# yondonfu/ai-rtc-agent

Measured on AMD Instinct MI355X. Metric: img2img FPS (SD-Turbo-class sd-turbo 512x512 1-step), higher is better.
Workload: dtype fp16; 1 GPU; model=sd-turbo (SD2.1-base UNet geometry, TAESD, 1-step), global_batch=1, resolution=512x512, parallelism=frame-level dp1, hip_graph=True

## Files before the change

### ai_rtc_agent_amd/ops/csrc/ext.cpp

```cpp

#include <torch/extension.h>
#include <ATen/cuda/CUDAContext.h>

#include "kernels.h"

#define CHECK_IN(x)                                                     \
  TORCH_CHECK(x.is_cuda(), #x " must be on GPU");                       \
  TORCH_CHECK(x.is_contiguous(), #x " must be contiguous")

namespace {

hipStream_t cur_stream() {
  return (hipStream_t)at::cuda::getCurrentCUDAStream().stream();
}

const uint16_t* h_ptr(const torch::Tensor& t) {
  return reinterpret_cast<const uint16_t*>(t.data_ptr<at::Half>());
}
uint16_t* h_ptr_mut(torch::Tensor& t) {
  return reinterpret_cast<uint16_t*>(t.data_ptr<at::Half>());
}

bool aligned16(const void* p) { return ((uintptr_t)p & 15) == 0; }

// ... 601 lines not shown
 public:
  VcnEncoder(int w, int h) : w_(w), h_(h) {
    char err[256] = {0};
    handle_ = airtc_vcn_enc_create(w, h, err, sizeof(err));
    if (!handle_) throw std::runtime_error(std::string("VCN encode: ") + err);
  }
  ~VcnEncoder() {
    if (handle_) airtc_vcn_enc_destroy(handle_);
  }
  VcnEncoder(const VcnEncoder&) = delete;
  pybind11::bytes encode(pybind11::bytes rgb, int qp) {
    std::string s(rgb);
    TORCH_CHECK((int)s.size() == w_ * h_ * 3, "rgb buffer size mismatch");
    std::vector<uint8_t> out((size_t)w_ * h_ * 2 + 65536);
    int n;
    {
      pybind11::gil_scoped_release nogil;
      n = airtc_vcn_enc_encode(handle_, (const uint8_t*)s.data(), qp,
                               out.data(), (int)out.size());
    }
    TORCH_CHECK(n > 0, "VCN encode failed rc=", n);
    return pybind11::bytes((const char*)out.data(), n);
  }

 private:
  void* handle_;
  int w_, h_;
};

pybind11::bytes h264_sps_pps(int width, int height) {
  uint8_t buf[256];
  int n = airtc_h264_sps_pps(width, height, buf, sizeof(buf));
  TORCH_CHECK(n > 0, "sps/pps generation failed");
  return pybind11::bytes(reinterpret_cast<const char*>(buf), n);
}

pybind11::dict vcn_probe() {
  char buf[512];
  int rc = airtc_vcn_probe(buf, sizeof(buf));
  pybind11::dict d;
  d["available"] = rc >= 0;
  d["h264_decode"] = rc >= 0 && (rc & 1);
  d["h264_encode"] = rc >= 0 && (rc & 2);
  d["detail"] = std::string(buf);
  return d;
}

torch::Tensor sched_add_noise(torch::Tensor x0, torch::Tensor noise,
                              torch::Tensor a, torch::Tensor bt) {
  CHECK_IN(x0);
  CHECK_IN(noise);
  TORCH_CHECK(x0.dtype() == torch::kHalf && noise.dtype() == torch::kHalf);
  TORCH_CHECK(a.dtype() == torch::kFloat && bt.dtype() == torch::kFloat);
  const long B = x0.size(0);
  TORCH_CHECK(a.numel() == B && bt.numel() == B, "coeffs must be (B,)");
  const long per_b = x0.numel() / B;
  TORCH_CHECK(per_b % 8 == 0, "row size must be a multiple of 8");
  auto out = torch::empty_like(x0);
  airtc_sched_add_noise(h_ptr(x0), h_ptr(noise), a.data_ptr<float>(),
                        bt.data_ptr<float>(), h_ptr_mut(out), per_b,
                        x0.numel(), cur_stream());
  return out;
}

torch::Tensor sched_blend(torch::Tensor xt, torch::Tensor eps,
                          torch::Tensor a, torch::Tensor bt,
                          torch::Tensor c_out, torch::Tensor c_skip) {
  CHECK_IN(xt);
  CHECK_IN(eps);
  TORCH_CHECK(xt.dtype() == torch::kHalf && eps.dtype() == torch::kHalf);
  const long B = xt.size(0);
  TORCH_CHECK(a.numel() == B && bt.numel() == B && c_out.numel() == B &&
              c_skip.numel() == B, "coeffs must be (B,)");
  const long per_b = xt.numel() / B;
  TORCH_CHECK(per_b % 8 == 0, "row size must be a multiple of 8");
  auto out = torch::empty_like(xt);
  airtc_sched_blend(h_ptr(xt), h_ptr(eps), a.data_ptr<float>(),
                    bt.data_ptr<float>(), c_out.data_ptr<float>(),
                    c_skip.data_ptr<float>(), h_ptr_mut(out), per_b,
                    xt.numel(), cur_stream());
  return out;
}

torch::Tensor rcfg_apply(int64_t mode, torch::Tensor eps, torch::Tensor coef,
                         c10::optional<torch::Tensor> delta,
                         c10::optional<torch::Tensor> stock, int64_t fbs) {
  CHECK_IN(eps);
  CHECK_IN(coef);
  TORCH_CHECK(mode >= 0 && mode <= 2, "mode must be 0 (self), 1 (initialize) or 2 (full)");
  TORCH_CHECK(eps.dtype() == torch::kHalf && coef.dtype() == torch::kFloat);
  TORCH_CHECK(eps.dim() >= 1 && fbs >= 1);
  const long B = coef.numel();
  const long rows_in = mode == 0 ? B : (mode == 1 ? B + fbs : 2 * B);
  TORCH_CHECK(B >= 1 && eps.size(0) == rows_in, "eps has ", eps.size(0),
              " rows, mode ", mode, " with ", B, " coefficient rows needs ",
              rows_in);
  TORCH_CHECK(fbs <= B && B % fbs == 0, "fbs must divide the row count");
  const long per_b = eps.numel() / rows_in;
  auto shape = eps.sizes().vec();
  shape[0] = B;
  auto out = torch::empty(shape, eps.options());
  auto overlap = [](const torch::Tensor& a, const torch::Tensor& b) {
    const char* a0 = static_cast<const char*>(a.data_ptr());
    const char* b0 = static_cast<const char*>(b.data_ptr());
    return a0 < b0 + b.nbytes() && b0 < a0 + a.nbytes();
  };
  TORCH_CHECK(!overlap(out, eps), "out must not alias eps");
  const float* dp = nullptr;
  uint16_t* sp = nullptr;
  bool vec = per_b % 8 == 0 && aligned16(eps.data_ptr()) &&
             aligned16(out.data_ptr());
  if (mode != 2) {
    TORCH_CHECK(delta.has_value() && stock.has_value(),
                "self/initialize need delta and stock");
    CHECK_IN((*delta));
    CHECK_IN((*stock));
    TORCH_CHECK(delta->dtype() == torch::kFloat && delta->numel() == B,
                "delta must be f32 (B,)");
    TORCH_CHECK(stock->dtype() == torch::kHalf && stock->sizes() == out.sizes(),
                "stock must be f16 with the output's shape");
    TORCH_CHECK(!overlap(*stock, eps), "stock must not alias eps");
    TORCH_CHECK(!overlap(out, *stock), "out must not alias stock");
    dp = delta->data_ptr<float>();
    sp = h_ptr_mut(*stock);
    vec = vec && aligned16(sp);
  }
  if (out.numel() == 0) return out;
  airtc_rcfg_apply((int)mode, h_ptr(eps), sp, coef.data_ptr<float>(), dp,
                   h_ptr_mut(out), B, fbs, per_b, vec ? 1 : 0, cur_stream());
  return out;
}

torch::Tensor conv2d_fp8(torch::Tensor x, torch::Tensor w_fp8,
                         torch::Tensor dq, double a_scale,
                         c10::optional<torch::Tensor> bias,
                         c10::optional<torch::Tensor> cbias,
                         c10::optional<torch::Tensor> residual, int64_t R,
                         int64_t S, int64_t stride, int64_t pad, int64_t act,
                         c10::optional<torch::Tensor> in_affine,
                         int64_t in_act, double out_scale) {
  CHECK_IN(x);
  CHECK_IN(w_fp8);
  CHECK_IN(dq);
  const bool x_q8 = x.dtype() == torch::kUInt8;
  TORCH_CHECK(x_q8 || x.dtype() == torch::kHalf,
              "x must be f16 or u8 e4m3 codes");
  TORCH_CHECK(w_fp8.dtype() == torch::kUInt8, "w_fp8 must be e4m3 bytes");
  TORCH_CHECK(dq.dtype() == torch::kFloat, "dq must be f32[OC]");
  const int B = x.size(0), H = x.size(1), W = x.size(2), IC = x.size(3);
  const int OC = w_fp8.size(0);
  TORCH_CHECK(IC % 64 == 0, "fp8 conv path requires IC % 64 == 0");
  TORCH_CHECK(dq.numel() == OC, "dq must have OC entries");
  TORCH_CHECK(w_fp8.size(1) == (long)R * S * IC, "w_fp8 must be (OC, R*S*IC)");
  TORCH_CHECK(!(x_q8 && in_affine.has_value()),
              "pre-quantized input cannot take a fused input affine");
  const int HO = (H + 2 * (int)pad - (int)R) / (int)stride + 1;
  const int WO = (W + 2 * (int)pad - (int)S) / (int)stride + 1;
  int path0 = airtc_conv2d_splitk_for(B, HO, WO, OC, IC);
  if (path0 == 0) path0 = HO * WO >= 2048 ? 1 : -1;
  const int splitk0 = path0 > 0 ? path0 : -path0;
  const bool want_q8 = out_scale > 0 && splitk0 == 1;
  auto out = torch::empty({B, HO, WO, OC},
                          x.options().dtype(want_q8 ? torch::kUInt8
                                                    : torch::kHalf));
  const float* bp = nullptr;
  if (bias.has_value()) {
    TORCH_CHECK(bias->dtype() == torch::kFloat && bias->is_contiguous());
    bp = bias->data_ptr<float>();
  }
  const uint16_t* cb = nullptr;
  if (cbias.has_value()) {
    CHECK_IN((*cbias));
    TORCH_CHECK(cbias->dtype() == torch::kHalf);
    cb = h_ptr(*cbias);
  }
  const uint16_t* res = nullptr;
  if (residual.has_value()) {
    CHECK_IN((*residual));
    TORCH_CHECK(residual->dtype() == torch::kHalf);
    TORCH_CHECK(residual->numel() == out.numel(), "residual shape mismatch");
    res = h_ptr(*residual);
  }
  const float* aff = nullptr;
  if (in_affine.has_value()) {
    CHECK_IN((*in_affine));
    TORCH_CHECK(in_affine->dtype() == torch::kFloat &&
                    in_affine->numel() == (long)B * IC * 2,
                "in_affine must be (B, IC, 2) f32");
    aff = in_affine->data_ptr<float>();
  }
  const int path = path0;
  const int splitk = splitk0;
  float* wsp = nullptr;
  torch::Tensor ws;
  if (splitk > 1) {
    ws = torch::empty({(long)B * splitk, (long)HO * WO, OC},
                      x.options().dtype(torch::kFloat));
    wsp = ws.data_ptr<float>();
  }
  const uint16_t* xp = x_q8
                           ? reinterpret_cast<const uint16_t*>(
                                 x.data_ptr<uint8_t>())
                           : h_ptr(x);
  uint16_t* op = want_q8 ? nullptr : h_ptr_mut(out);
  uint8_t* oq = want_q8 ? out.data_ptr<uint8_t>() : nullptr;
  airtc_conv2d_fp8_mfma(xp, w_fp8.data_ptr<uint8_t>(),
                        dq.data_ptr<float>(), bp, cb, res, op, wsp,
                        B, H, W, IC, HO, WO, OC, (int)R, (int)S, (int)stride,
                        (int)pad, (int)act, path, aff, (int)in_act,
                        (float)a_scale, x_q8 ? 1 : 0, oq,
                        want_q8 ? (float)(1.0 / out_scale) : 0.f,
                        cur_stream());
  return out;
}

torch::Tensor fp8_mx_probe(torch::Tensor A, torch::Tensor B, int64_t sa,
                           int64_t sb) {
  CHECK_IN(A);
  CHECK_IN(B);
  TORCH_CHECK(A.dtype() == torch::kUInt8 && B.dtype() == torch::kUInt8);
  TORCH_CHECK(A.numel() == 2048 && B.numel() == 2048, "fragments are 2048B");
  auto draw = torch::empty({256}, A.options().dtype(torch::kFloat));
  airtc_fp8_mx_probe(A.data_ptr<uint8_t>(), B.data_ptr<uint8_t>(),
                     draw.data_ptr<float>(), (int)sa, (int)sb, cur_stream());
  return draw;
}

torch::Tensor fp8_quant_probe(torch::Tensor in16, double sa, int64_t variant) {
  CHECK_IN(in16);
  TORCH_CHECK(in16.dtype() == torch::kHalf && in16.numel() == 16);
  auto out = torch::empty({16}, in16.options().dtype(torch::kUInt8));
  airtc_fp8_quant_probe(h_ptr(in16), (float)sa, out.data_ptr<uint8_t>(),
                        (int)variant, cur_stream());
  return out;
}

pybind11::tuple fp8_cvt_probe(torch::Tensor fin, double scale,
                              torch::Tensor enc_in) {
  CHECK_IN(fin);
  CHECK_IN(enc_in);
  TORCH_CHECK(fin.dtype() == torch::kHalf && fin.numel() == 2);
  TORCH_CHECK(enc_in.dtype() == torch::kUInt8 && enc_in.numel() == 2);
  auto enc_out = torch::empty({2}, enc_in.options());
  auto dec_out = torch::empty({2}, fin.options());
  airtc_fp8_cvt_probe(h_ptr(fin), (float)scale, enc_out.data_ptr<uint8_t>(),
                      enc_in.data_ptr<uint8_t>(), h_ptr_mut(dec_out),
                      cur_stream());
  return pybind11::make_tuple(enc_out, dec_out);
}

}

void airtc_register_dtls(pybind11::module_& m);

torch::Tensor airtc_linear_residual(const torch::Tensor& x,
                                    const torch::Tensor& weight,
                                    const c10::optional<torch::Tensor>& bias,
                                    const torch::Tensor& residual);

PYBIND11_MODULE(TORCH_EXTENSION_NAME, m) {
  airtc_register_dtls(m);
  m.def("linear_residual", &airtc_linear_residual,
        "x (...,K) · weight (N,K)ᵀ + bias (N,) + residual in one hipBLASLt "
        "call (bias epilogue, C = residual, beta = 1); contiguous f16, fp32 "
        "accumulation",
        pybind11::arg("x"), pybind11::arg("weight"), pybind11::arg("bias"),
        pybind11::arg("residual"));
  m.attr("LT_NO_ALGORITHM") = "linear_residual: no hipBLASLt algorithm";
  m.def("conv2d", &conv2d, "implicit-GEMM MFMA conv2d (NHWC)",
        pybind11::arg("x"), pybind11::arg("w_perm"), pybind11::arg("bias"),
        pybind11::arg("cbias"), pybind11::arg("residual"), pybind11::arg("R"),
        pybind11::arg("S"), pybind11::arg("stride"), pybind11::arg("pad"),
        pybind11::arg("act"), pybind11::arg("in_affine") = pybind11::none(),
        pybind11::arg("in_act") = 0, pybind11::arg("x2") = pybind11::none(),
        pybind11::arg("upsample2x") = false);
  m.def("conv2d_tinyic", &conv2d_tinyic,
        "tiny-IC conv (IC <= 4, K <= 36), lanes along OC (NHWC)",
        pybind11::arg("x"), pybind11::arg("w_tiny"), pybind11::arg("bias"),
        pybind11::arg("cbias"), pybind11::arg("residual"), pybind11::arg("R"),
        pybind11::arg("S"), pybind11::arg("stride"), pybind11::arg("pad"),
        pybind11::arg("act"));
  m.def("conv2d_stats", &conv2d_stats,
        "conv2d that also returns GroupNorm partials of its output for a "
        "consumer norm with stats_groups groups: (out, partials | None)",
        pybind11::arg("x"), pybind11::arg("w_perm"), pybind11::arg("bias"),
        pybind11::arg("cbias"), pybind11::arg("residual"), pybind11::arg("R"),
        pybind11::arg("S"), pybind11::arg("stride"), pybind11::arg("pad"),
        pybind11::arg("act"), pybind11::arg("in_affine"),
        pybind11::arg("in_act"), pybind11::arg("stats_groups"),
        pybind11::arg("x2") = pybind11::none(),
        pybind11::arg("upsample2x") = false);
  m.def("group_norm_silu", &group_norm_silu, pybind11::arg("x"),
        pybind11::arg("groups"), pybind11::arg("gamma"), pybind11::arg("beta"),
        pybind11::arg("eps"), pybind11::arg("act"),
        pybind11::arg("partials") = pybind11::none());
  m.def("group_norm_silu_fp8", &group_norm_silu_fp8,
        "GN+act writing e4m3 codes (producer-side fp8 quantization)",
        pybind11::arg("x"), pybind11::arg("groups"), pybind11::arg("gamma"),
        pybind11::arg("beta"), pybind11::arg("eps"), pybind11::arg("act"),
        pybind11::arg("a_scale"),
        pybind11::arg("partials") = pybind11::none());
  m.def("group_norm_coeffs", &group_norm_coeffs,
        "(B,C,2) f32 affine pairs for the fused GN->conv input transform");
  m.def("layer_norm", &layer_norm);
  m.def("attention_bhlc", &attention_bhlc);
  m.def("silu", &silu);
  m.def("geglu", &geglu);
  m.def("add_act", &add_act);
  m.def("upsample2x", &upsample2x);
  m.def("sched_add_noise", &sched_add_noise,
        "fused q(x_t|x0) sample: a*x0 + b*noise (per-batch-row coeffs)");
  m.def("sched_blend", &sched_blend,
        "fused LCM step: c_out*(x_t - b*eps)/a + c_skip*x_t");
  m.def("rcfg_apply", &rcfg_apply,
        "residual-CFG step, per-row f32 coefficients; shifts stock in place");
  m.def("preprocess_u8", &preprocess_u8);
  m.def("postprocess_u8", &postprocess_u8);
  m.def("fit_resize_u8", &fit_resize_u8,
        "crop + antialiased resize of a u8 RGB frame into one slot");
  m.def("fit_resize_u8_i420", &fit_resize_u8_i420,
        "crop + antialiased resize of a u8 RGB frame into a whole I420 frame");
  m.def("rgb_u8_to_i420", &rgb_u8_to_i420,
        "(B,H,W,3) u8 RGB -> (B,3H/2,W) u8 I420 (BT.601 limited, integer)",
        pybind11::arg("x"), pybind11::arg("out") = pybind11::none());
  m.def("postprocess_i420", &postprocess_i420,
        "(B,H,W,3) f16 in [-1,1] -> (B,3H/2,W) u8 I420 in one kernel",
        pybind11::arg("img"), pybind11::arg("out") = pybind11::none());
  m.def("i420_to_rgb_u8", &i420_to_rgb_u8,
        "(B,3H/2,W) u8 I420 -> (B,H,W,3) u8 RGB",
        pybind11::arg("x"), pybind11::arg("out") = pybind11::none());
  m.def("canny_hint", &canny_hint,
        "(B,H,W,3) u8 RGB -> edge hint written into out (f16/f32); thr (B,2) "
        "i32 read on the device, hysteresis bounded to `reach` steps",
        pybind11::arg("frames"), pybind11::arg("thr"), pybind11::arg("reach"),
        pybind11::arg("out"));
  m.def("conv2d_fp8", &conv2d_fp8,
        "fp8 e4m3 implicit-GEMM conv2d on the MX-scaled MFMA (NHWC)",
        pybind11::arg("x"), pybind11::arg("w_fp8"), pybind11::arg("dq"),
        pybind11::arg("a_scale"), pybind11::arg("bias"),
        pybind11::arg("cbias"), pybind11::arg("residual"), pybind11::arg("R"),
        pybind11::arg("S"), pybind11::arg("stride"), pybind11::arg("pad"),
        pybind11::arg("act"), pybind11::arg("in_affine") = pybind11::none(),
        pybind11::arg("in_act") = 0, pybind11::arg("out_scale") = 0.0);
  m.def("fp8_mx_probe", &fp8_mx_probe,
        "raw-fragment v_mfma_scale_f32_16x16x128_f8f6f4 tile (layout probe)");
  m.def("fp8_quant_probe", &fp8_quant_probe,
        "conv kernel's exact 16-value activation encode (variant 0/1)");
  m.def("fp8_cvt_probe", &fp8_cvt_probe,
        "v_cvt_scalef32_pk_{fp8_f16,f16_fp8} semantics probe");
  m.def("vcn_probe", &vcn_probe, "probe the VCN VA-API stack");
  m.def("h264_sps_pps", &h264_sps_pps, "Annex-B SPS+PPS for (w, h)");
  m.def("h264sw_table_check", []() { return airtc_h264sw_table_check(); },
        "0 iff all CAVLC tables are prefix-free");
  pybind11::class_<H264SwEncoder>(m, "H264SwEncoder")
      .def(pybind11::init<int, int, int, int>(), pybind11::arg("w"),
           pybind11::arg("h"), pybind11::arg("slices") = 4,
           pybind11::arg("mb_mode") = 0)
      .def("encode", &H264SwEncoder::encode, pybind11::arg("rgb"),
           pybind11::arg("qp"), pybind11::arg("keyframe") = true,
           "RGB24 bytes + QP -> Annex-B (IDR, or P when keyframe=false)")
      .def("encode_yuv", &H264SwEncoder::encode_yuv, pybind11::arg("i420"),
           pybind11::arg("qp"), pybind11::arg("keyframe") = true,
           "tight I420 bytes + QP -> Annex-B, no colour conversion");
  m.def("h264_pred4",
        [](int mode, pybind11::bytes top, pybind11::bytes left, int tl,
           bool ht, bool hl, bool htl) {
          std::string t(top), l(left);
          TORCH_CHECK(t.size() == 8 && l.size() == 4, "t8/l4 sizes");
          uint8_t out[16];
          airtc_h264_pred4(mode, (const uint8_t*)t.data(),
                           (const uint8_t*)l.data(), (uint8_t)tl, ht, hl, htl,
                           out);
          return pybind11::bytes((const char*)out, 16);
        },
        "one 4x4 intra prediction (decoder path) for golden tests");
  pybind11::class_<H264SwDecoder>(m, "H264SwDecoder")
      .def(pybind11::init<>())
      .def("decode", &H264SwDecoder::decode,
           "Annex-B AU -> (rgb bytes, w, h) | None")
      .def("decode_yuv", &H264SwDecoder::decode_yuv,
           "Annex-B AU -> (i420 bytes, w, h, is_i420) | None");
  pybind11::class_<VcnEncoder>(m, "VcnEncoder")
      .def(pybind11::init<int, int>())
      .def("encode", &VcnEncoder::encode,
           "RGB24 bytes + QP -> Annex-B IDR via the VCN hardware encoder");
}
```

### ai_rtc_agent_amd/ops/csrc/kernels.h

```cpp
#pragma once

#include <hip/hip_runtime.h>
#include <stdint.h>

extern "C" {

void airtc_preprocess_u8(const uint8_t* in, uint16_t* out, long n, hipStream_t s);
void airtc_postprocess_u8(const uint16_t* in, uint8_t* out, long n, hipStream_t s);
void airtc_silu_f16(const uint16_t* in, uint16_t* out, long n, hipStream_t s);
void airtc_geglu_f16(const uint16_t* in, uint16_t* out, long rows, long inner,
                     hipStream_t s);
void airtc_add_act_f16(const uint16_t* a, const uint16_t* b, uint16_t* out,
                       long n, int act, hipStream_t s);
void airtc_upsample2x_f16(const uint16_t* in, uint16_t* out, int B, int H,
                          int W, int C, hipStream_t s);
void airtc_fit_resize_u8(const uint8_t* src, int Ws, uint8_t* dst, int H,
                         int W, int y0, int x0, int ch, int cw, int oy,
                         int ox, int oh, int ow, hipStream_t s);
void airtc_fit_resize_u8_i420(const uint8_t* src, int Ws, uint8_t* dst, int H,
                              int W, int y0, int x0, int ch, int cw,
                              hipStream_t s);
void airtc_rgb_u8_to_i420(const uint8_t* in, uint8_t* out, int B, int H,
                          int W, hipStream_t s);
void airtc_postprocess_i420(const uint16_t* in, uint8_t* out, int B, int H,
                            int W, hipStream_t s);
void airtc_i420_to_rgb_u8(const uint8_t* in, uint8_t* out, int B, int H,
                          int W, hipStream_t s);
int airtc_canny_hint(const uint8_t* in, const int* thr, void* out,
                     int out_f32, int B, int H, int W, int reach,
                     hipStream_t s);
void airtc_sched_add_noise(const uint16_t* x0, const uint16_t* noise,
                           const float* a, const float* bt, uint16_t* out,
                           long per_b, long n, hipStream_t s);
void airtc_sched_blend(const uint16_t* xt, const uint16_t* eps,
                       const float* a, const float* bt, const float* c_out,
                       const float* c_skip, uint16_t* out, long per_b, long n,
                       hipStream_t s);
void airtc_rcfg_apply(int mode, const uint16_t* eps, uint16_t* stock,
                      const float* gm1, const float* delta, uint16_t* out,
                      long B, long fbs, long per_b, int vec, hipStream_t s);

#define AIRTC_GN_MAX_PART 64
int airtc_group_norm_nchunk(int B, int G);
void airtc_group_norm(const uint16_t* x, const float* part, int npart,
                      const float* gamma, const float* beta, uint16_t* out,
                      uint8_t* out_q8, float* ws, int B, int HW, int C, int G,
                      float eps, int act, float a_scale, hipStream_t s);
void airtc_layer_norm(const uint16_t* x, const float* gamma, const float* beta,
                      uint16_t* out, long rows, int C, float eps,
                      hipStream_t s);
void airtc_group_norm_coeffs(const uint16_t* x, const float* gamma,
                             const float* beta, float* coeffs, float* ws,
                             int B, int HW, int C, int G, float eps,
                             hipStream_t s);

int airtc_conv2d_splitk_for(int B, int HO, int WO, int OC, int IC);
int airtc_conv2d_mfma(const uint16_t* x, const uint16_t* w, const float* bias,
                      const uint16_t* cbias, const uint16_t* residual,
                      uint16_t* out, float* ws, int B, int H, int W, int IC,
                      int HO, int WO, int OC, int R, int S, int stride,
                      int pad, int act, int path, const float* in_aff,
                      int in_act, float* gn_part, int gn_groups,
                      const uint16_t* x2, int IC2, int up, hipStream_t s);
int airtc_conv2d_tinyic_ok(int IC, int R, int S);
void airtc_conv2d_tinyic(const uint16_t* x, const float* wt, const float* bias,
                         const uint16_t* cbias, const uint16_t* residual,
                         uint16_t* out, int B, int H, int W, int IC, int HO,
                         int WO, int OC, int R, int S, int stride, int pad,
                         int act, hipStream_t s);
int airtc_conv2d_stats_nchunk(int B, int HO, int WO, int OC, int IC, int G,
                              int act);
void airtc_conv2d_direct(const uint16_t* x, const uint16_t* w,
                         const float* bias, const uint16_t* cbias,
                         const uint16_t* residual, uint16_t* out, int B, int H,
                         int W, int IC, int HO, int WO, int OC, int R, int S,
                         int stride, int pad, int act, const float* in_aff,
                         int in_act, hipStream_t s);

void airtc_conv2d_fp8_mfma(const uint16_t* x, const uint8_t* w_fp8,
                           const float* dq, const float* bias,
                           const uint16_t* cbias, const uint16_t* residual,
                           uint16_t* out, float* ws, int B, int H, int W,
                           int IC, int HO, int WO, int OC, int R, int S,
                           int stride, int pad, int act, int path,
                           const float* in_aff, int in_act, float a_scale,
                           int x_is_q8, uint8_t* out_q8, float out_inv,
                           hipStream_t s);
void airtc_fp8_mx_probe(const uint8_t* A, const uint8_t* B, float* draw,
                        int sa, int sb, hipStream_t s);
void airtc_fp8_cvt_probe(const uint16_t* fin, float scale, uint8_t* enc_out,
                         const uint8_t* enc_in, uint16_t* dec_out,
                         hipStream_t s);
void airtc_fp8_quant_probe(const uint16_t* in16, float sa, uint8_t* out16,
                           int variant, hipStream_t s);

void airtc_attention(const uint16_t* q, const uint16_t* k, const uint16_t* v,
                     uint16_t* out, int B, int H, int Lq, int Lk, int d,
                     long q_sb, long q_sh, long q_row, long k_sb, long k_sh,
                     long k_row, long o_sb, long o_sh, long o_row, float scale,
                     hipStream_t s);

}

extern "C" int airtc_vcn_probe(char* buf, int buflen);

extern "C" int airtc_h264_sps_pps(int width, int height, uint8_t* buf,
                                  int buflen);
```

### ai_rtc_agent_amd/ops/csrc/norms.hip

```cpp

#include <stdlib.h>

#include "common.h"

typedef __attribute__((__vector_size__(2 * sizeof(_Float16)))) _Float16 f16x2;

__device__ __forceinline__ void gn_chunk_range(long n2, int chunk, int nchunk,
                                               long* lo, long* hi) {
  const long per = (n2 + nchunk - 1) / nchunk;
  *lo = (long)chunk * per;
  *hi = min(n2, *lo + per);
}

__global__ void group_norm_stats_kernel(const f16* __restrict__ x,
                                        float* __restrict__ ws, int HW, int C,
                                        int G, int nchunk) {
  const int chunk = blockIdx.y;
  const int b = blockIdx.x / G;
  const int g = blockIdx.x % G;
  const int Cg = C / G;
  const int Cg2 = Cg / 2;
  const long base = (long)b * HW * C + (long)g * Cg;
  long lo, hi;
  gn_chunk_range((long)HW * Cg2, chunk, nchunk, &lo, &hi);

  float sum = 0.f, sumsq = 0.f;
  for (long i = lo + threadIdx.x; i < hi; i += blockDim.x) {
    long p = i / Cg2, c2 = i - p * Cg2;
    f16x2 v = *reinterpret_cast<const f16x2*>(&x[base + p * C + c2 * 2]);
    float a = (float)v[0], c = (float)v[1];
    sum += a + c;
    sumsq += a * a + c * c;
  }
  __shared__ float red[2][4];
  int lane = threadIdx.x & 63, wid = threadIdx.x >> 6;
  sum = wave_reduce(sum, SumOp());
  sumsq = wave_reduce(sumsq, SumOp());
  if (lane == 0) { red[0][wid] = sum; red[1][wid] = sumsq; }
  __syncthreads();
  if (threadIdx.x == 0) {
    float s0 = 0.f, s1 = 0.f;
    for (int i = 0; i < (int)(blockDim.x >> 6); ++i) { s0 += red[0][i]; s1 += red[1][i]; }
    float* w = &ws[((long)blockIdx.x * nchunk + chunk) * 2];
    w[0] = s0;
    w[1] = s1;
  }
}

__device__ __forceinline__ void gn_fold_partials(const float* w, int npart,
                                                 float n, float eps,
                                                 float* mean_out,
                                                 float* rstd_out) {
  float s0 = 0.f, s1 = 0.f;
  for (int i = 0; i < npart; ++i) { s0 += w[2 * i]; s1 += w[2 * i + 1]; }
  const float mean = s0 / n;
  *mean_out = mean;
  *rstd_out = rsqrtf(s1 / n - mean * mean + eps);
}

template <bool Q8>
__global__ void group_norm_apply_kernel(
    const f16* __restrict__ x, const float* __restrict__ ws,
    const float* __restrict__ gamma, const float* __restrict__ beta,
    f16* __restrict__ out, uint8_t* __restrict__ outq, int HW, int C, int G,
    int nchunk, float eps, int act, float inv_sa) {
  const int chunk = blockIdx.y;
  const int b = blockIdx.x / G;
  const int g = blockIdx.x % G;
  const int Cg = C / G;
  const int Cg2 = Cg / 2;
  const long base = (long)b * HW * C + (long)g * Cg;

  __shared__ float stats[2];
  if (threadIdx.x == 0)
    gn_fold_partials(&ws[(long)blockIdx.x * nchunk * 2], nchunk,
                     (float)HW * Cg, eps, &stats[0], &stats[1]);
  __syncthreads();
  const float mean = stats[0], rstd = stats[1];

  long lo, hi;
  gn_chunk_range((long)HW * Cg2, chunk, nchunk, &lo, &hi);
  for (long i = lo + threadIdx.x; i < hi; i += blockDim.x) {
    long p = i / Cg2, c2 = i - p * Cg2;
    long idx = base + p * C + c2 * 2;
    f16x2 v = *reinterpret_cast<const f16x2*>(&x[idx]);
    int ch = g * Cg + (int)c2 * 2;
    float a[2];
#pragma unroll
    for (int j = 0; j < 2; ++j) {
      float t = ((float)v[j] - mean) * rstd * gamma[ch + j] + beta[ch + j];
      a[j] = apply_act(t, act);
    }
    if (Q8) {
#pragma unroll
      for (int j = 0; j < 2; ++j)
        a[j] = fminf(fmaxf(a[j] * inv_sa, -448.0f), 448.0f);
      int p2 = __builtin_amdgcn_cvt_pk_fp8_f32(a[0], a[1], 0, false);
      *reinterpret_cast<short*>(&outq[idx]) = (short)(p2 & 0xFFFF);
    } else {
      v[0] = (f16)a[0];
      v[1] = (f16)a[1];
      *reinterpret_cast<f16x2*>(&out[idx]) = v;
    }
  }
}

extern "C" int airtc_group_norm_nchunk(int B, int G) {
  int n = (int)(512 / max(1, B * G));
  if (n < 1) n = 1;
  if (n > 64) n = 64;
  return n;
}

struct GnPlan { int gpt, ct, pt; };

static bool gn_fast_plan(int C, int G, GnPlan* p) {
  if (G <= 0 || C % 8 != 0 || C % G != 0) return false;
  const int Cg = C / G;
  int gpt = 0;
  for (int d = 1; d <= G && d <= 64; ++d)
    if (G % d == 0 && (d * Cg) % 8 == 0 && d * Cg <= 512) gpt = d;
  if (!gpt) return false;
  p->gpt = gpt;
  p->ct = gpt * Cg / 8;
  p->pt = 256 / p->ct;
  return true;
}

__global__ __launch_bounds__(256) void group_norm_stats_v8_kernel(
    const f16* __restrict__ x, float* __restrict__ part, int HW, int C, int G,
    int ct, int per) {
  __shared__ float red[2][2048];
  __shared__ float col[2][512];
  const int cx = threadIdx.x % ct, py = threadIdx.x / ct;
  const int pt = 256 / ct;
  const int cw = ct * 8;
  const int b = blockIdx.z;
  const int p_lo = blockIdx.x * per;
  const int p_hi = min(HW, p_lo + per);
  if (py < pt) {
    float s[8], q[8];
#pragma unroll
    for (int j = 0; j < 8; ++j) s[j] = q[j] = 0.f;
    const f16* xp = x + ((long)b * HW + p_lo + py) * C + blockIdx.y * cw + cx * 8;
    const long step = (long)pt * C;
#pragma unroll 2
    for (int p = p_lo + py; p < p_hi; p += pt, xp += step) {
      const f16x8 v = *reinterpret_cast<const f16x8*>(xp);
#pragma unroll
      for (int j = 0; j < 8; ++j) {
        const float f = (float)v[j];
        s[j] += f;
        q[j] += f * f;
      }
    }
#pragma unroll
    for (int j = 0; j < 8; ++j) {
      red[0][py * cw + cx * 8 + j] = s[j];
      red[1][py * cw + cx * 8 + j] = q[j];
    }
  }
  __syncthreads();
  for (int c = threadIdx.x; c < cw; c += 256) {
    float a0 = 0.f, a1 = 0.f;
    for (int r = 0; r < pt; ++r) {
      a0 += red[0][r * cw + c];
      a1 += red[1][r * cw + c];
    }
    col[0][c] = a0;
    col[1][c] = a1;
  }
  __syncthreads();
  const int Cg = C / G;
  const int gpt = cw / Cg;
  if ((int)threadIdx.x < gpt) {
    float a0 = 0.f, a1 = 0.f;
    for (int i = 0; i < Cg; ++i) {
      a0 += col[0][threadIdx.x * Cg + i];
      a1 += col[1][threadIdx.x * Cg + i];
    }
    const int g = blockIdx.y * gpt + threadIdx.x;
    float* w = part + (((long)b * G + g) * gridDim.x + blockIdx.x) * 2;
    w[0] = a0;
    w[1] = a1;
  }
}

template <bool Q8>
__global__ __launch_bounds__(256) void group_norm_apply_v8_kernel(
    const f16* __restrict__ x, const float* __restrict__ part,
    const float* __restrict__ gamma, const float* __restrict__ beta,
    f16* __restrict__ out, uint8_t* __restrict__ outq, int HW, int C, int G,
    int npart, float eps, int act, float inv_sa, int ct, int per) {
  __shared__ float gst[2][64];
  __shared__ float tab[2][512];
  const int cx = threadIdx.x % ct, py = threadIdx.x / ct;
  const int pt = 256 / ct;
  const int cw = ct * 8;
  const int b = blockIdx.z;
  const int ch0 = blockIdx.y * cw;
  const int Cg = C / G;
  const int gpt = cw / Cg;
  if ((int)threadIdx.x < gpt) {
    const int g = blockIdx.y * gpt + threadIdx.x;
    gn_fold_partials(&part[((long)b * G + g) * npart * 2], npart,
                     (float)HW * Cg, eps, &gst[0][threadIdx.x],
                     &gst[1][threadIdx.x]);
  }
  __syncthreads();
  for (int c = threadIdx.x; c < cw; c += 256) {
    const int gi = c / Cg;
    const float sc = gamma[ch0 + c] * gst[1][gi];
    tab[0][c] = sc;
    tab[1][c] = beta[ch0 + c] - gst[0][gi] * sc;
  }
  __syncthreads();
  if (py >= pt) return;
  float sc[8], sh[8];
#pragma unroll
  for (int j = 0; j < 8; ++j) {
    sc[j] = tab[0][cx * 8 + j];
    sh[j] = tab[1][cx * 8 + j];
  }
  const int p_lo = blockIdx.x * per;
  const int p_hi = min(HW, p_lo + per);
  long idx = ((long)b * HW + p_lo + py) * C + ch0 + cx * 8;
  const long step = (long)pt * C;
#pragma unroll 2
  for (int p = p_lo + py; p < p_hi; p += pt, idx += step) {
    f16x8 v = *reinterpret_cast<const f16x8*>(&x[idx]);
    if (Q8) {
      float a[8];
#pragma unroll
      for (int j = 0; j < 8; ++j) {
        const float t = (float)v[j] * sc[j] + sh[j];
        a[j] = fminf(fmaxf(apply_act(t, act) * inv_sa, -448.0f), 448.0f);
      }
      int w0 = __builtin_amdgcn_cvt_pk_fp8_f32(a[0], a[1], 0, false);
      w0 = __builtin_amdgcn_cvt_pk_fp8_f32(a[2], a[3], w0, true);
      int w1 = __builtin_amdgcn_cvt_pk_fp8_f32(a[4], a[5], 0, false);
      w1 = __builtin_amdgcn_cvt_pk_fp8_f32(a[6], a[7], w1, true);
      uint2 q;
      q.x = (uint32_t)w0;
      q.y = (uint32_t)w1;
      *reinterpret_cast<uint2*>(&outq[idx]) = q;
    } else {
#pragma unroll
      for (int j = 0; j < 8; ++j)
        v[j] = (f16)apply_act((float)v[j] * sc[j] + sh[j], act);
      *reinterpret_cast<f16x8*>(&out[idx]) = v;
    }
  }
}

static int gn_launch_stats_v8(const GnPlan& pl, const f16* x, float* part,
                              int B, int HW, int C, int G, hipStream_t s) {
  const int n0 = min(64, ceil_div(HW, pl.pt));
  const int per = ceil_div(HW, n0);
  const int npart = ceil_div(HW, per);
  hipLaunchKernelGGL(group_norm_stats_v8_kernel, dim3(npart, G / pl.gpt, B),
                     dim3(256), 0, s, x, part, HW, C, G, pl.ct, per);
  return npart;
}

static void gn_launch_apply_v8(const GnPlan& pl, const f16* x,
                               const float* part, int npart,
                               const float* gamma, const float* beta, f16* out,
                               uint8_t* outq, int B, int HW, int C, int G,
                               float eps, int act, float inv_sa,
                               hipStream_t s) {
  const int tiles = G / pl.gpt;
  int nch = ceil_div(512, tiles * B);
  nch = max(1, min(nch, ceil_div(HW, pl.pt)));
  const int per = ceil_div(HW, nch);
  dim3 grid(ceil_div(HW, per), tiles, B);
  if (outq)
    hipLaunchKernelGGL(group_norm_apply_v8_kernel<true>, grid, dim3(256), 0, s,
                       x, part, gamma, beta, out, outq, HW, C, G, npart, eps,
                       act, inv_sa, pl.ct, per);
  else
    hipLaunchKernelGGL(group_norm_apply_v8_kernel<false>, grid, dim3(256), 0,
                       s, x, part, gamma, beta, out, outq, HW, C, G, npart,
                       eps, act, inv_sa, pl.ct, per);
}

static bool gn_fast_ok(const void* x, const void* out, int B, int C, int G,
                       GnPlan* pl) {
  const char* e = getenv("AIRTC_GN_FAST");
  if (!(e && atoi(e) == 1) || B > 65535) return false;
  if ((((uintptr_t)x | (uintptr_t)out) & 15) != 0) return false;
  return gn_fast_plan(C, G, pl);
}

__global__ void group_norm_coeffs_kernel(const float* __restrict__ ws,
                                         const float* __restrict__ gamma,
                                         const float* __restrict__ beta,
                                         float* __restrict__ coeffs, int HW,
                                         int C, int G, int nchunk,
                                         float eps) {
  const int b = blockIdx.x / G;
  const int g = blockIdx.x % G;
  const int Cg = C / G;
  __shared__ float stats[2];
  if (threadIdx.x == 0)
    gn_fold_partials(&ws[(long)blockIdx.x * nchunk * 2], nchunk,
                     (float)HW * Cg, eps, &stats[0], &stats[1]);
  __syncthreads();
  const float mean = stats[0], rstd = stats[1];
  for (int c = threadIdx.x; c < Cg; c += blockDim.x) {
    const int ch = g * Cg + c;
    const float sc = gamma[ch] * rstd;
    float* o = &coeffs[((long)b * C + ch) * 2];
    o[0] = sc;
    o[1] = beta[ch] - mean * sc;
  }
}

extern "C" void airtc_group_norm_coeffs(const uint16_t* x, const float* gamma,
                                        const float* beta, float* coeffs,
                                        float* ws, int B, int HW, int C,
                                        int G, float eps, hipStream_t s) {
  const int nchunk = airtc_group_norm_nchunk(B, G);
  dim3 grid(B * G, nchunk);
  hipLaunchKernelGGL(group_norm_stats_kernel, grid, dim3(256), 0, s,
                     reinterpret_cast<const f16*>(x), ws, HW, C, G, nchunk);
  hipLaunchKernelGGL(group_norm_coeffs_kernel, dim3(B * G), dim3(256), 0, s,
                     ws, gamma, beta, coeffs, HW, C, G, nchunk, eps);
}

extern "C" void airtc_group_norm(const uint16_t* x, const float* part,
                                 int npart, const float* gamma,
                                 const float* beta, uint16_t* out,
                                 uint8_t* out_q8, float* ws, int B, int HW,
                                 int C, int G, float eps, int act,
                                 float a_scale, hipStream_t s) {
  const f16* xp = reinterpret_cast<const f16*>(x);
  f16* op = reinterpret_cast<f16*>(out);
  const float inv_sa = out_q8 ? 1.0f / a_scale : 0.f;
  GnPlan pl;
  const bool fast = gn_fast_ok(
      x, out_q8 ? (const void*)out_q8 : (const void*)out, B, C, G, &pl);
  if (!part) {
    if (fast) {
      npart = gn_launch_stats_v8(pl, xp, ws, B, HW, C, G, s);
    } else {
      npart = airtc_group_norm_nchunk(B, G);
      hipLaunchKernelGGL(group_norm_stats_kernel, dim3(B * G, npart),
                         dim3(256), 0, s, xp, ws, HW, C, G, npart);
    }
    part = ws;
  }
  if (fast) {
    gn_launch_apply_v8(pl, xp, part, npart, gamma, beta, op, out_q8, B, HW, C,
                       G, eps, act, inv_sa, s);
    return;
  }
  dim3 grid(B * G, npart);
  if (out_q8)
    hipLaunchKernelGGL(group_norm_apply_kernel<true>, grid, dim3(256), 0, s,
                       xp, part, gamma, beta, op, out_q8, HW, C, G, npart, eps,
                       act, inv_sa);
  else
    hipLaunchKernelGGL(group_norm_apply_kernel<false>, grid, dim3(256), 0, s,
                       xp, part, gamma, beta, op, out_q8, HW, C, G, npart, eps,
                       act, inv_sa);
}

__global__ void layer_norm_kernel(const f16* __restrict__ x,
                                  const float* __restrict__ gamma,
                                  const float* __restrict__ beta,
                                  f16* __restrict__ out, long rows, int C8,
                                  float eps) {
  const int lane = threadIdx.x & 63;
  const long row = (long)blockIdx.x * (blockDim.x >> 6) + (threadIdx.x >> 6);
  if (row >= rows) return;
  const f16x8* xr = reinterpret_cast<const f16x8*>(x) + row * C8;

  float sum = 0.f, sumsq = 0.f;
  for (int i = lane; i < C8; i += WAVE) {
    f16x8 v = xr[i];
#pragma unroll
    for (int j = 0; j < 8; ++j) {
      float f = (float)v[j];
      sum += f;
      sumsq += f * f;
    }
  }
  sum = wave_reduce(sum, SumOp());
  sumsq = wave_reduce(sumsq, SumOp());
  float n = (float)C8 * 8.0f;
  float mean = sum / n;
  float rstd = rsqrtf(sumsq / n - mean * mean + eps);

  f16x8* orow = reinterpret_cast<f16x8*>(out) + row * C8;
  for (int i = lane; i < C8; i += WAVE) {
    f16x8 v = xr[i];
#pragma unroll
    for (int j = 0; j < 8; ++j)
      v[j] = (f16)(((float)v[j] - mean) * rstd * gamma[i * 8 + j] + beta[i * 8 + j]);
    orow[i] = v;
  }
}

extern "C" void airtc_layer_norm(const uint16_t* x, const float* gamma,
                                 const float* beta, uint16_t* out, long rows,
                                 int C, float eps, hipStream_t s) {
  int waves_per_block = 4;
  long blocks = (rows + waves_per_block - 1) / waves_per_block;
  hipLaunchKernelGGL(layer_norm_kernel, dim3((uint32_t)blocks),
                     dim3(waves_per_block * WAVE), 0, s,
                     reinterpret_cast<const f16*>(x), gamma, beta,
                     reinterpret_cast<f16*>(out), rows, C / 8, eps);
}
```

Measured before the change: 156.0 frames/s.

## Add single-launch register-resident GroupNorm kernel for small groups

Adds a one-launch GroupNorm path for f16 calls without precomputed partials or fp8 output, used when the fast v8 path is off. One 1024-thread block per (batch, group) loads the group into registers, computes mean and a two-pass variance with block reductions, then normalizes and writes. This replaces the separate stats and apply launches and avoids re-reading the input from memory. It is gated by an env var that defaults on, and by a per-thread load bucket; with few groups (B*G<256) the gate is zero, so it applies only when there are many groups. The risk is low occupancy and register pressure at larger load counts.

```diff
diff --git a/ai_rtc_agent_amd/ops/csrc/ext.cpp b/ai_rtc_agent_amd/ops/csrc/ext.cpp
--- a/ai_rtc_agent_amd/ops/csrc/ext.cpp
+++ b/ai_rtc_agent_amd/ops/csrc/ext.cpp
@@ -927,6 +927,17 @@
         pybind11::arg("partials") = pybind11::none());
   m.def("group_norm_coeffs", &group_norm_coeffs,
         "(B,C,2) f32 affine pairs for the fused GN->conv input transform");
+  m.def(
+      "group_norm_onepass_plan",
+      [](int64_t B, int64_t HW, int64_t C, int64_t G) {
+        const int64_t lim = INT32_MAX;
+        if (B > lim || HW > lim || C > lim || G > lim) return 0;
+        return airtc_group_norm_onepass_plan((int)B, (int)HW, (int)C, (int)G);
+      },
+      "loads-per-thread bucket of the one-launch GroupNorm for an f16 call "
+      "without partials, 0 = stats + apply pair (reads AIRTC_GN_ONEPASS)",
+      pybind11::arg("B"), pybind11::arg("HW"), pybind11::arg("C"),
+      pybind11::arg("G"));
   m.def("layer_norm", &layer_norm);
   m.def("attention_bhlc", &attention_bhlc);
   m.def("silu", &silu);
diff --git a/ai_rtc_agent_amd/ops/csrc/kernels.h b/ai_rtc_agent_amd/ops/csrc/kernels.h
--- a/ai_rtc_agent_amd/ops/csrc/kernels.h
+++ b/ai_rtc_agent_amd/ops/csrc/kernels.h
@@ -46,6 +46,7 @@
                       const float* gamma, const float* beta, uint16_t* out,
                       uint8_t* out_q8, float* ws, int B, int HW, int C, int G,
                       float eps, int act, float a_scale, hipStream_t s);
+int airtc_group_norm_onepass_plan(int B, int HW, int C, int G);
 void airtc_layer_norm(const uint16_t* x, const float* gamma, const float* beta,
                       uint16_t* out, long rows, int C, float eps,
                       hipStream_t s);
diff --git a/ai_rtc_agent_amd/ops/csrc/norms.hip b/ai_rtc_agent_amd/ops/csrc/norms.hip
--- a/ai_rtc_agent_amd/ops/csrc/norms.hip
+++ b/ai_rtc_agent_amd/ops/csrc/norms.hip
@@ -292,6 +292,158 @@
   return gn_fast_plan(C, G, pl);
 }
 
+#define GN_OP_THREADS 1024
+#define GN_OP_MAX_NL 64
+#define GN_OP_MAX_CG 256
+#define GN_OP_GATE_NL_FEW 0
+#define GN_OP_GATE_NL_FULL 64
+
+__device__ __forceinline__ uint32_t gn_op_pixel(uint32_t i, uint32_t magic) {
+  return __umulhi(i << 1, magic);
+}
+
+static uint32_t gn_op_magic(uint32_t Cg2) { return (1u << 31) / Cg2 + 1u; }
+
+__device__ __forceinline__ uint32_t gn_op_tid() {
+  uint32_t t = threadIdx.x;
+  asm volatile("" : "+v"(t));
+  return t;
+}
+
+__device__ __forceinline__ f16x2 gn_op_fresh(f16x2 v) {
+  uint32_t w = __builtin_bit_cast(uint32_t, v);
+  asm volatile("" : "+v"(w));
+  return __builtin_bit_cast(f16x2, w);
+}
+
+__device__ __forceinline__ float gn_op_block_sum(float v, float* red) {
+  v = wave_reduce(v, SumOp());
+  if ((threadIdx.x & 63) == 0) red[threadIdx.x >> 6] = v;
+  __syncthreads();
+  float s = 0.f;
+#pragma unroll
+  for (int i = 0; i < GN_OP_THREADS / WAVE; ++i) s += red[i];
+  return s;
+}
+
+template <int NL>
+__global__ __launch_bounds__(GN_OP_THREADS) void group_norm_onepass_kernel(
+    const f16* __restrict__ x, const float* __restrict__ gamma,
+    const float* __restrict__ beta, f16* __restrict__ out, int HW, int C,
+    int G, uint32_t magic, float eps, int act) {
+  __shared__ float red[2][GN_OP_THREADS / WAVE];
+  __shared__ float gb[2][GN_OP_MAX_CG];
+  const int b = blockIdx.x / G;
+  const int g = blockIdx.x % G;
+  const int Cg = C / G;
+  const uint32_t Cg2 = Cg >> 1;
+  const uint32_t n2 = (uint32_t)HW * Cg2;
+  const uint32_t skip = 2u * (uint32_t)(C - Cg);
+  const long base = (long)b * HW * C + (long)g * Cg;
+  const char* xg = reinterpret_cast<const char*>(x + base);
+  char* og = reinterpret_cast<char*>(out + base);
+
+  f16x2 v[NL];
+  uint32_t tid = gn_op_tid();
+#pragma unroll
+  for (int k = 0; k < NL; ++k) {
+    v[k][0] = v[k][1] = (f16)0.f;
+    if ((uint32_t)k * GN_OP_THREADS < n2) {
+      const uint32_t i = min(tid + k * GN_OP_THREADS, n2 - 1);
+      v[k] = *reinterpret_cast<const f16x2*>(
+          xg + (4 * i + gn_op_pixel(i, magic) * skip));
+    }
+  }
+  if ((int)threadIdx.x < Cg) {
+    gb[0][threadIdx.x] = gamma[g * Cg + threadIdx.x];
+    gb[1][threadIdx.x] = beta[g * Cg + threadIdx.x];
+  }
+
+  float s0 = 0.f, s1 = 0.f;
+  tid = gn_op_tid();
+#pragma unroll
+  for (int k = 0; k < NL; ++k) {
+    const uint32_t i = tid + k * GN_OP_THREADS;
+    s0 += i < n2 ? (float)v[k][0] : 0.f;
+    s1 += i < n2 ? (float)v[k][1] : 0.f;
+  }
+  const float n = (float)HW * (float)Cg;
+  const float mean = gn_op_block_sum(s0 + s1, red[0]) / n;
+
+  float q0 = 0.f, q1 = 0.f;
+  tid = gn_op_tid();
+#pragma unroll
+  for (int k = 0; k < NL; ++k) {
+    const uint32_t i = tid + k * GN_OP_THREADS;
+    const f16x2 h = gn_op_fresh(v[k]);
+    const float d0 = (float)h[0] - mean, d1 = (float)h[1] - mean;
+    q0 += i < n2 ? d0 * d0 : 0.f;
+    q1 += i < n2 ? d1 * d1 : 0.f;
+  }
+  const float rstd = rsqrtf(gn_op_block_sum(q0 + q1, red[1]) / n + eps);
+
+  tid = gn_op_tid();
+#pragma unroll
+  for (int k = 0; k < NL; ++k) {
+    const uint32_t i = tid + k * GN_OP_THREADS;
+    if (i < n2) {
+      const uint32_t p = gn_op_pixel(i, magic);
+      const uint32_t c = 2 * (i - p * Cg2);
+      const f16x2 h = gn_op_fresh(v[k]);
+      f16x2 o;
+#pragma unroll
+      for (int j = 0; j < 2; ++j) {
+        const float t =
+            ((float)h[j] - mean) * rstd * gb[0][c + j] + gb[1][c + j];
+        o[j] = (f16)apply_act(t, act);
+      }
+      *reinterpret_cast<f16x2*>(og + (4 * i + p * skip)) = o;
+    }
+  }
+}
+
+extern "C" int airtc_group_norm_onepass_plan(int B, int HW, int C, int G) {
+  const char* e = getenv("AIRTC_GN_ONEPASS");
+  const int mode = e ? atoi(e) : 1;
+  if (mode == 0) return 0;
+  if (B <= 0 || HW <= 0 || G <= 0 || C <= 0 || C % G != 0) return 0;
+  const int Cg = C / G;
+  if (Cg % 2 != 0 || Cg > GN_OP_MAX_CG) return 0;
+  if ((long)HW * C >= (1L << 31) || (long)B * G >= (1L << 31)) return 0;
+  const long n2 = (long)HW * (Cg / 2);
+  const long need = (n2 + GN_OP_THREADS - 1) / GN_OP_THREADS;
+  if (need > GN_OP_MAX_NL) return 0;
+  if (mode != 2) {
+    const long limit = (long)B * G >= 256 ? GN_OP_GATE_NL_FULL
+                                          : GN_OP_GATE_NL_FEW;
+    if (need > limit) return 0;
+  }
+  int nl = 4;
+  while (nl < need) nl *= 2;
+  return nl;
+}
+
+static void gn_launch_onepass(int nl, const f16* x, const float* gamma,
+                              const float* beta, f16* out, int B, int HW,
+                              int C, int G, float eps, int act,
+                              hipStream_t s) {
+  const uint32_t magic = gn_op_magic((uint32_t)(C / G / 2));
+  const dim3 grid(B * G), block(GN_OP_THREADS);
+#define GN_OP_CASE(N)                                                        \
+  case N:                                                                    \
+    hipLaunchKernelGGL(group_norm_onepass_kernel<N>, grid, block, 0, s, x,   \
+                       gamma, beta, out, HW, C, G, magic, eps, act);         \
+    break;
+  switch (nl) {
+    GN_OP_CASE(4)
+    GN_OP_CASE(8)
+    GN_OP_CASE(16)
+    GN_OP_CASE(32)
+    GN_OP_CASE(64)
+  }
+#undef GN_OP_CASE
+}
+
 __global__ void group_norm_coeffs_kernel(const float* __restrict__ ws,
                                          const float* __restrict__ gamma,
                                          const float* __restrict__ beta,
@@ -340,6 +492,13 @@
   GnPlan pl;
   const bool fast = gn_fast_ok(
       x, out_q8 ? (const void*)out_q8 : (const void*)out, B, C, G, &pl);
+  if (!part && !out_q8 && !fast) {
+    const int nl = airtc_group_norm_onepass_plan(B, HW, C, G);
+    if (nl) {
+      gn_launch_onepass(nl, xp, gamma, beta, op, B, HW, C, G, eps, act, s);
+      return;
+    }
+  }
   if (!part) {
     if (fast) {
       npart = gn_launch_stats_v8(pl, xp, ws, B, HW, C, G, s);
```

Result: no change. 155.8 frames/s (-0.2%).
